# nikhilTkur/Multigrid_dolfinx

Measured on AMD Instinct MI355X. Metric: V-cycles/sec + achieved HBM GB/s, 3D Poisson P1 1024³ DoF, 1/2/4/8 MI355X, higher is better.
Workload: dtype f64; 1 GPU; 3D Poisson P1, 6-level 1024^3 fine grid, 1076890625 DoF, V(50,50) weighted Jacobi omega=0.6667, injection, Q1 prolongation, exact block-LU coarsest solve, explicit zeros pruned (7-point rows); levels=6, dim=3, elements_per_dim=1024, parallelism=single

## Files before the change

multigrid_dolfinx_amd/csrc/mg_capi.hip:

```cpp
#include "../../include/mg_hip.h"
#include "mg_csr_check.h"
#include "mg_kernels.hip.h"
#include "mg_direct.hip.h"
#include "mg_jacobi2.hip.h"
#include "mg_jacobik3d.hip.h"
#include "mg_jacobiblk.hip.h"
#include "mg_lattice.hip.h"
#include "mg_diffusion_mf.hip.h"
#include "mg_diffusion_mf_batch.hip.h"
#include "mg_diffusion_adj.hip.h"
#include "mg_diffusion_flux.hip.h"
#include "mg_diffusion_points.hip.h"
#include "mg_diffusion_kappa.hip.h"

#include <dlfcn.h>
#include <rccl/rccl.h>

#include <algorithm>
#include <array>
#include <cmath>
#include <cstdio>
#include <cstdlib>
#include <cstring>
#include <initializer_list>
// ... 121 lines not shown
    int64_t rep_escape = 0;
    int cls_halo = 0;
    bool flat = false;
    int W = 0, R = 1;
    int64_t nslices = 0;
    DevBuf<double> vals;
    DevBuf<int> cols;
    DevBuf<unsigned long long> codes;
    DevBuf<int> offsets;
    int ntable = 0, dcode = 0;
    bool coded = false;
    bool rb_ok = false;
    int mc_ok = -1;
    DevBuf<double> dvals;
    bool sdia = false;
    int wu = 0;
    int up[8] = {0, 0, 0, 0, 0, 0, 0, 0};
    int64_t mlead = 0, mslices = 0;
    DevBuf<unsigned char> cls;
    DevBuf<double> ctab;
    int ncls = 0;
    DevBuf<unsigned char> scls;
    DevBuf<int> s_off;
    DevBuf<double> s_val;
    DevBuf<int> s_cnt;
    int nscls = 0;
    DevBuf<int> s_pack;
    int lm_ntop = 0;
    int lm_top[LM_K] = {0, 0, 0, 0, 0, 0, 0, 0};
    struct MarchPlan {
        DevBuf<int> iv;
        int64_t waves[2] = {0, 0}, planes[2] = {0, 0};
    };
    MarchPlan plan[6];
    int cmain = 0;
    double cm[8] = {0, 0, 0, 0, 0, 0, 0, 0};
    int64_t cls_lead = 0;
    DevBuf<double> dinv;
    bool mf = false;
    DevBuf<double> kappa;
    int faces = MG_FACES_ALL;
    bool diffusion_hierarchy = false;
    bool react = false;
    DevBuf<double> rdiag;
    int robin = 0;
    DVector v, v2, f, err, ftrue;
    DVector sw;
    DVector fcg_x, fcg_p, fcg_q, fcg_b;
    bool cheb_est_ok = false;
    double cheb_lmax_est = 0.0, cheb_user_lmin = 0.0, cheb_user_lmax = 0.0;
    DevBuf<int> perm;
    int p1_ok = -1;
    std::vector<int> h_offsets;
    unsigned long long nnz_stored = 0, nnz_nonzero = 0;
    std::vector<int> splits;
};

}

struct DirectSolver {
    bool tried = false, ok = false;
    BtGeom g{};
    DevBuf<double> T;
    DevBuf<int> lcol, ucol;
    DevBuf<double> lval, uval;
    DevBuf<double> y, x, w;
};
// ... 76 lines not shown
    DevBuf<double> alpha[6];
    int alpha_N = 0;
    int dkappa_gather = 0;
    int lattice_tile = 0;
    int lattice_segments = 0;
    int slab_pair_form = 0;
    int graph_comm = 0;
    uint64_t epoch = 1;
    std::vector<CycleGraph> graphs;
    bool capturing = false;
    int use_direct = 1;
    int require_diagonal = 1;
    int fuse_restrict = 1;
    int fuse_block = 1;
    int64_t fuse_block_min_rows = (int64_t)1 << 15, fuse_block_max_rows = (int64_t)1 << 23;
    int fuse_block_k = 0, fuse_block_ez = 11;
    int direct_block_rows = 2048;
    int fuse_2d_lines = 0;
    int gen_odd_rows = 0;
    int cls_escape = 1;
    int storage_auto = 1;
    int storage_qbits = 0;
    int use_classes = 1;
    int fuse_sweeps = 1;
    int64_t fuse_min_rows = (int64_t)1 << 24;
    int fuse_segments = 0;
    int fuse_nontemporal = 0;
    int fuse_classes = 1;
    int fuse_plain_shape = 0;
    int fuse_plain = 2;
    int class_sweeps = 1;
    int fuse_k = 5;
    int fuse_k_shape = -1;
    int fuse_k_segments = 0;
    int timing_force_form = -1;
    int64_t fuse_k_slab_min_rows = (int64_t)1 << 20;
    int fuse_k_slab_min_sweeps = 4;
    int64_t fuse_k_min_rows = (int64_t)1 << 24;
    int64_t fuse_k_small_rows = (int64_t)1 << 22;
    int64_t fuse_k5_min_rows = (int64_t)1 << 26;
    int64_t fuse_k4_min_rows = 0;
    int fuse_k_nt_store = 0;
    int fuse_k_min_side = 32;
    int fuse_k_tail = 1;
    int fuse_k_small_tiles = 0;
    int fuse_k_pf = 1;
    int fuse_k_dpp = 1;
    int fuse_k_plan = 1;
    std::vector<const void*> large_lds_kernels;
    int fuse_shape = 1;
    int fuse_wi = 0;
    int fuse_even = 0;
    int march_sweeps = 1;
    int64_t march_min_rows = (int64_t)1 << 22;
    int march_shape = 0;
    int64_t fuse_small_2d_rows = 2048;
    int fuse_small = 1;
    int fuse_2d = 1;
    int fuse_2d_k = 5;
    int fuse_xcd_chunk = 32;
    int cls_blocks_per_cu = 4;
    DirectSolver direct;
    DevTemp ptab_count;
    int p1_prolong = 0;
    DevTemp rtab_count;
    DevTemp rtab_off;
// ... 1199 lines not shown
template <int K>
int escape_window_k(mg_context* c, const Level& L, const unsigned char* cls, int64_t clead, unsigned* most) {
    constexpr int WI = 64 - 2 * K, HY = 16 * 2 - 2 * K + 2;
    JK3WindowArgs a{};
    a.cls = cls; a.clead = clead; a.P = L.g.plane; a.nx = L.g.nx; a.ny = L.g.ny; a.nz = L.g.nk;
    a.ntx = (a.nx + WI - 1) / WI; a.nty = (a.ny + HY - 1) / HY;
    a.most = reinterpret_cast<unsigned*>(c->partials.get());
    HIP_TRY(hipMemsetAsync(a.most, 0, sizeof(unsigned), c->stream));
    hipLaunchKernelGGL((jk3_escape_window<K, 16, 2, 1>), dim3((unsigned)(a.ntx * a.nty)), dim3(256), 0, c->stream, a);
    HIP_TRY(hipGetLastError());
    HIP_TRY(hipMemcpyAsync(most, a.most, sizeof(unsigned), hipMemcpyDeviceToHost, c->stream));
    HIP_TRY(hipStreamSynchronize(c->stream));
    if (std::getenv("MG_DEBUG_STORAGE"))
        std::fprintf(stderr, "[mg] escape rows: at most %u in %d planes of a tile (%d sweeps per pass, pool of %d)\n", *most, K + 2, K, jk3_pool(K));
    return 0;
}

int escape_kmax(mg_context* c, const Level& L, const unsigned char* cls, int64_t clead, int* kmax) {
    *kmax = 0;
    if (L.wu != 4 || L.g.nk < 8 || L.g.nx < 32 || L.g.ny < 32) return 0;
    unsigned most = 0;
    MG_TRY(escape_window_k<5>(c, L, cls, clead, &most));
    if (most <= (unsigned)jk3_pool(5)) { *kmax = 5; return 0; }
    MG_TRY(escape_window_k<4>(c, L, cls, clead, &most));
    if (most <= (unsigned)jk3_pool(4)) { *kmax = 4; return 0; }
    MG_TRY(escape_window_k<3>(c, L, cls, clead, &most));
    if (most <= (unsigned)jk3_pool(3)) *kmax = 3;
    return 0;
}

struct JK3Range { int za0, za1, zb0, zb1; };

int jk3_shape(const mg_context* c, int K) {
    return c->fuse_k_shape >= 0 ? c->fuse_k_shape : (K >= 5 ? 8 : 7);
}

int jk3_shape_for(const mg_context* c, int K, int ncls) {
    return jk3_shape(c, K) >= 3 && ncls > 64 ? 1 : jk3_shape(c, K);
}

int march_plan_slot(const mg_context* c, const Level& L, int K) {
    if (!c->fuse_k_plan || !c->fuse_k_dpp || K < 3 || K > 5 || !L.cls || L.cls_escape || is_slab(c, L)) return -1;
    const int shape = jk3_shape_for(c, K, L.ncls);
    return shape == 7 || shape == 8 ? (K - 3) * 2 + (shape - 7) : -1;
}

int ensure_march_plan(mg_context* c, Level& L, int K, int slot) {
    Level::MarchPlan& mp = L.plan[slot];
    if (mp.iv) return 0;
    JK3PlanArgs a{};
    a.cls = L.cls; a.clead = L.cls_lead; a.P = L.g.plane; a.nx = L.g.nx; a.ny = L.g.ny; a.nz = L.g.nk; a.cmain = L.cmain;
    const int WI = 64 - 2 * K, HY = 32 - 2 * K + 2;
    a.ntx = (a.nx + WI - 1) / WI; a.nty = (a.ny + HY - 1) / HY;
    const size_t n = (size_t)a.ntx * a.nty * 16 * 4;
    DevBuf<int> iv;
    MG_TRY(iv.alloc(c, n));
    a.plan = iv;
    with_int<3, 4, 5>(K, [&](auto k) { hipLaunchKernelGGL((jk3_plan<decltype(k)::value, 16, 2, 1>), dim3((unsigned)(a.ntx * a.nty)), dim3(16 * WAVE), 0, c->stream, a); });
    HIP_TRY(hipGetLastError());
    std::vector<int> h(n);
    HIP_TRY(hipMemcpyAsync(h.data(), iv, n * sizeof(int), hipMemcpyDeviceToHost, c->stream));
    HIP_TRY(hipStreamSynchronize(c->stream));
    for (size_t i = 0; i < n; i += 4) {
        if (h[i + 1] > h[i]) { ++mp.waves[0]; mp.planes[0] += h[i + 1] - h[i]; }
        if (h[i + 3] > h[i + 2] && (h[i + 2] != h[i] || h[i + 3] != h[i + 1])) { ++mp.waves[1]; mp.planes[1] += h[i + 3] - h[i + 2]; }
    }
    mp.iv = std::move(iv);
    return 0;
}

template <int K, int NW, int LPW, int M, bool DPP, int PF = 1, int WPE = (NW == 12 ? 3 : 2), int TR = 256, bool ESC = false, bool B1 = false>
int launch_jacobikc_t(mg_context* c, JK3Args a, bool finest, const JK3Range& zr, int seglen) {
    constexpr int EX = 64 * M, EY = NW * LPW, WI = EX - 2 * K, HY = EY - 2 * K + 2;
    a.ntx = (a.nx + WI - 1) / WI;
    a.nty = (a.ny + HY - 1) / HY;
    const int64_t ntile = (int64_t)a.ntx * a.nty;
    constexpr size_t lds = B1 ? jk3b_lds_bytes<K, NW, LPW, M, TR>() : jk3_lds_bytes<K, NW, LPW, M, TR, ESC>();
    static_assert(lds <= 160 * 1024, "one CU's LDS");
    a.za0 = zr.za0; a.za1 = zr.za1; a.zb0 = zr.zb0; a.zb1 = zr.zb1;
    const int planes = std::max(0, zr.za1 - zr.za0) + std::max(0, zr.zb1 - zr.zb0);
    if (planes <= 0) return 0;
    a.ta = (int)ntile; a.seglen_b = 1;
    int64_t items = 0;
    if (seglen <= 0) {
        int64_t cus = std::max(1, c->prop.multiProcessorCount) * (int64_t)std::max<size_t>(1, std::min<size_t>(160 * 1024 / lds, (size_t)(4 * WPE / NW)));
        if (c->fuse_k_tail > 1) cus = c->fuse_k_tail;
        const double warm = 1.4 * K;
        int best = 1, best_ta = (int)ntile, best_m = 1;
        double best_cost = 1e300;
        const bool tail = c->fuse_k_tail && zr.zb1 <= zr.zb0;
        for (int n = 1; n <= std::max(1, planes / 8); ++n) {
            const int len = (planes + n - 1) / n;
            const int64_t full = ntile * n / cus;
            int64_t ta = tail ? std::min<int64_t>(ntile, full * cus / n) : ntile;
            if (ta <= 0 || (ntile - ta) * 2 > cus) ta = ntile;
            const int64_t tb = ntile - ta;
            const int m = tb > 0 ? (int)std::max<int64_t>(1, std::min<int64_t>(cus / tb, planes / 4)) : 1;
            const double cost = (double)((ta * n + cus - 1) / cus) * (len + warm) + (tb > 0 ? (planes + m - 1) / m + warm : 0.0);
            if (cost < best_cost) { best_cost = cost; best = n; best_ta = (int)ta; best_m = m; }
        }
        if (c->fuse_k_segments > 0) { best = std::min(c->fuse_k_segments, planes); best_ta = (int)ntile; }
        seglen = (planes + best - 1) / best;
        a.ta = best_ta;
        a.seglen_b = best_ta < ntile ? (planes + best_m - 1) / best_m : 1;
    }
    a.seglen = seglen;
    {
        const int nseg = (std::max(0, zr.za1 - zr.za0) + seglen - 1) / seglen + (std::max(0, zr.zb1 - zr.zb0) + seglen - 1) / seglen;
        items = (int64_t)a.ta * nseg;
        if (a.ta < ntile) items += (ntile - a.ta) * (int64_t)((planes + a.seglen_b - 1) / a.seglen_b);
    }
    a.xcd_chunk = (unsigned)c->fuse_xcd_chunk;
    unsigned grid = 0;
    MG_TRY(tile_grid(items, a.xcd_chunk, &grid));
    a.nitems = (unsigned)items;
    if (a.ncls > TR) return fail("more row classes than this tile shape keeps in LDS");
    void (*kern)(JK3Args) = nullptr;
    if constexpr (ESC) kern = sdia_jacobikc_escape<K, NW, LPW, M, DPP, PF, WPE, TR>;
    else if constexpr (B1) kern = finest ? sdia_jacobikc_finest_b1<K, NW, LPW, M, WPE, TR> : sdia_jacobikc_b1<K, NW, LPW, M, WPE, TR>;
    else kern = finest ? sdia_jacobikc_finest<K, NW, LPW, M, DPP, PF, WPE, TR> : sdia_jacobikc<K, NW, LPW, M, DPP, PF, WPE, TR>;
    MG_TRY(allow_large_lds(c, reinterpret_cast<const void*>(kern), lds));
    hipLaunchKernelGGL(kern, dim3(grid), dim3(NW * WAVE), lds, c->stream, a);
    HIP_TRY(hipGetLastError());
    c->jk3_tail = a.ta < ntile ? 1 : 0;
    return 0;
}

template <int K, int PF>
int launch_jacobikc_kp(mg_context* c, const JK3Args& a, bool finest, const JK3Range& zr, int seglen) {
    if (!c->fuse_k_dpp) return launch_jacobikc_t<K, 12, 2, 2, false, PF>(c, a, finest, zr, seglen);
    int shape = jk3_shape_for(c, K, a.ncls);
    if (shape == 1 && a.ncls <= 64 && K <= 4 && c->fuse_k_small_tiles) {
        constexpr int WI = 64 - 2 * K, HY = 48 - 2 * K + 2;
        if ((int64_t)((a.nx + WI - 1) / WI) * ((a.ny + HY - 1) / HY) < std::max(1, c->prop.multiProcessorCount)) shape = 4;
    }
    switch (shape) {
        case 1: return launch_jacobikc_t<K, 12, 4, 1, true, PF>(c, a, finest, zr, seglen);
        case 2: return launch_jacobikc_t<K, 8, 3, 2, true, PF>(c, a, finest, zr, seglen);
        case 3: return launch_jacobikc_t<K, 6, 4, 1, true, PF, 3, 64>(c, a, finest, zr, seglen);
        case 4: return launch_jacobikc_t<K, 8, 3, 1, true, PF, 4, 64>(c, a, finest, zr, seglen);
        case 5: if constexpr (K <= 4) return launch_jacobikc_t<K, 4, 6, 1, true, PF, 2, 64>(c, a, finest, zr, seglen);
        case 6: if constexpr (K <= 4 && PF == 1) return launch_jacobikc_t<K, 16, 3, 1, true, 1, 4>(c, a, finest, zr, seglen);
        case 7: return launch_jacobikc_t<K, 16, 2, 1, true, PF, 4>(c, a, finest, zr, seglen);
        case 8: if constexpr (PF == 1) return launch_jacobikc_t<K, 16, 2, 1, true, 1, 4, 256, false, true>(c, a, finest, zr, seglen);
                else return fail("tile shape 8 stages one plane of x (fuse_k_pf 1)");
        default: return launch_jacobikc_t<K, 12, 2, 2, true, PF>(c, a, finest, zr, seglen);
    }
}

template <int K>
int launch_jacobikc_k(mg_context* c, const JK3Args& a, bool finest, const JK3Range& zr, int seglen) {
    if (a.escape) {
        if constexpr (K >= 3) return launch_jacobikc_t<K, 16, 2, 1, true, 1, 4, 256, true>(c, a, finest, zr, seglen);
        else return fail("levels with escape rows take three to five sweeps per pass");
    }
    if constexpr (K == 3 || K == 4) {
        if (c->fuse_k_pf == 2 && (K == 3 || jk3_shape(c, K) == 7)) return launch_jacobikc_kp<K, 2>(c, a, finest, zr, seglen);
    }
    if constexpr (K == 2) return launch_jacobikc_t<K, 12, 4, 1, true, 1>(c, a, finest, zr, seglen);
    else return launch_jacobikc_kp<K, 1>(c, a, finest, zr, seglen);
}

int launch_jacobikc(mg_context* c, Level& L, int K, const double* x_rows, const double* f_rows, double* out_rows,
                    const JK3Range* zr = nullptr, int seglen = 0) {
    JK3Args a{};
    a.x = x_rows; a.f = f_rows; a.out = out_rows;
    fill_classes_lead(a, L);
    a.P = L.g.plane; a.nx = L.g.nx; a.ny = L.g.ny; a.nz = L.g.nk; a.omega = c->omega;
    const bool dist = is_slab(c, L);
    a.plo = dist && c->comm.rank > 0 ? K : 0;
    a.phi = dist && c->comm.rank + 1 < c->comm.world ? K : 0;
    if (dist && (L.hd < K || L.cls_halo != 1)) return fail("the level's halos are not prepared for that many sweeps per pass");
    if (L.cls_escape && K > L.esc_kmax) return fail("too many escape rows per tile for that many sweeps per pass");
    a.force_form = c->timing_force_form;
    a.nt_store = c->fuse_k_nt_store;
    if (const int slot = march_plan_slot(c, L, K); slot >= 0 && a.force_form < 0 && !zr) {
        if (!L.plan[slot].iv) {
            hipStreamCaptureStatus st = hipStreamCaptureStatusNone;
            HIP_TRY(hipStreamIsCapturing(c->stream, &st));
            if (st == hipStreamCaptureStatusNone) MG_TRY(ensure_march_plan(c, L, K, slot));
        }
        a.plan = L.plan[slot].iv;
    }
    a.escape = L.cls_escape ? 1 : 0; a.dvals = L.dvals; a.mlead = L.mlead; a.sshift = L.R == 1 ? 6 : (L.R == 2 ? 7 : 8);
    const JK3Range whole{0, L.g.nk, 0, 0};
    c->jk3_tail = 0;
    int rc = 0;
    if (!with_int<2, 3, 4, 5>(K, [&](auto k) { rc = launch_jacobikc_k<decltype(k)::value>(c, a, is_finest(c, L), zr ? *zr : whole, seglen); }))
        return fail("sweeps per pass must be in 2..5");
    return rc;
}

int check_coloring(mg_context* c, Level& L) {
    MG_TRY(need_stored_rows(c, L, "the colouring check of the Gauss-Seidel smoothers"));
    EllArgs a{};
    a.vals = L.vals; a.cols = L.cols; a.codes = L.codes; a.offsets = L.offsets; a.W = L.W;
    a.nloc = L.nloc; a.lead = L.g.lead; a.dinv = L.dinv; a.color_kind = COLOR_LATTICE9; a.grow0 = L.row0; a.gnx = L.g.nx; a.gny = L.g.ny;
    int* d_flag = reinterpret_cast<int*>(c->partials.get());
    HIP_TRY(hipMemsetAsync(d_flag, 0, sizeof(int), c->stream));
    const dim3 grid(blocks_for(L.nloc, 256)), blk(256);
    if (L.sdia) {
        a.vals = L.dvals; a.mlead = L.mlead;
        for (int t = 0; t < 8; ++t) a.up[t] = L.up[t];
        with_int_else<4, 1, 2>(L.R, [&](auto r) { hipLaunchKernelGGL(sdia_check_coloring<decltype(r)::value>, grid, blk, 0, c->stream, a, L.wu, d_flag); });
    } else {
        with_int_else<4, 1, 2>(L.R, [&](auto r) { hipLaunchKernelGGL(ell_check_coloring<decltype(r)::value>, grid, blk, 0, c->stream, a, L.nslices, d_flag); });
    }
    HIP_TRY(hipGetLastError());
    int flag = 1;
    HIP_TRY(hipMemcpyAsync(&flag, d_flag, sizeof(int), hipMemcpyDeviceToHost, c->stream));
    HIP_TRY(hipStreamSynchronize(c->stream));
    L.mc_ok = flag ? 0 : 1;
    return 0;
}

bool sweeps2d_ok(const mg_context* c, const Level& L) {
    if (!c->fuse_2d || !L.sdia || L.wu != 3 || !cls_full(L) || !c->fuse_classes || L.flat || !L.replicated) return false;
    return L.g.ny == 1 && L.up[1] == 1 && L.up[2] == L.g.nx && L.g.nx >= 8 && L.g.nz >= 8;
}

template <int K, int H>
// ... 2477 lines not shown
        c->lattice_march_min_rows = value;
    } else if (k == "dkappa_gather") {
        c->dkappa_gather = value != 0;
    } else if (k == "lattice_gs2") {
        c->lattice_gs2 = value != 0;
    } else if (k == "lattice_tile") {
        if (value < 0 || value > 2) return fail("lattice_tile must be 0, 1 or 2");
        c->lattice_tile = (int)value;
    } else if (k == "lattice_segments") {
        if (value < 0 || value > 4096) return fail("lattice_segments must be in 0..4096");
        c->lattice_segments = (int)value;
    } else if (k == "fuse_xcd_chunk") {
        if (value < 1 || value > 512) return fail("fuse_xcd_chunk must be in 1..512");
        c->fuse_xcd_chunk = (int)value;
    } else if (k == "cls_blocks_per_cu") {
        if (value < 1 || value > 64) return fail("cls_blocks_per_cu must be in 1..64");
        c->cls_blocks_per_cu = (int)value;
    } else if (k == "fuse_wi") {
        c->fuse_wi = (int)value;
    } else if (k == "fuse_even") {
        c->fuse_even = value != 0;
    } else if (k == "class_sweeps") {
        c->class_sweeps = value != 0;
    } else if (k == "fuse_plain_shape") {
        if (value < 0 || value > 2) return fail("fuse_plain_shape must be 0..2");
        c->fuse_plain_shape = (int)value;
    } else if (k == "fuse_plain") {
        if (value != 1 && value != 2) return fail("fuse_plain must be 1 or 2");
        c->fuse_plain = (int)value;
    } else if (k == "fuse_k") {
        if (value < 0 || value > 5) return fail("fuse_k must be in 0..5 (below 3: pairs of sweeps only)");
        c->fuse_k = (int)value;
    } else if (k == "fuse_k_shape") {
        if (value < -1 || value > 8) return fail("fuse_k_shape must be 0..8, or -1 (by sweeps per pass)");
        c->fuse_k_shape = (int)value;
    } else if (k == "fuse_k_slab_min_rows") {
        c->fuse_k_slab_min_rows = value;
    } else if (k == "fuse_k_slab_min_sweeps") {
        if (value < 2) return fail("fuse_k_slab_min_sweeps must be at least 2");
        c->fuse_k_slab_min_sweeps = (int)value;
    } else if (k == "fuse_k_min_rows") {
        c->fuse_k_min_rows = value;
    } else if (k == "fuse_k_small_rows") {
        c->fuse_k_small_rows = value;
    } else if (k == "fuse_k5_min_rows") {
        c->fuse_k5_min_rows = value;
    } else if (k == "fuse_k4_min_rows") {
        c->fuse_k4_min_rows = value;
    } else if (k == "fuse_k_nt_store") {
        c->fuse_k_nt_store = value != 0;
    } else if (k == "fuse_k_min_side") {
        if (value < 16 || value > 32) return fail("fuse_k_min_side must be in 16..32");
        c->fuse_k_min_side = (int)value;
    } else if (k == "fuse_k_tail") {
        if (value < 0) return fail("fuse_k_tail must be >= 0");
        c->fuse_k_tail = (int)value;
    } else if (k == "fuse_k_small_tiles") {
        c->fuse_k_small_tiles = value != 0;
    } else if (k == "fuse_k_pf") {
        if (value != 1 && value != 2) return fail("fuse_k_pf must be 1 or 2");
        c->fuse_k_pf = (int)value;
    } else if (k == "fuse_k_dpp") {
        c->fuse_k_dpp = value != 0;
    } else if (k == "fuse_k_plan") {
        c->fuse_k_plan = value != 0;
    } else if (k == "fuse_k_segments") {
        if (value < 0) return fail("fuse_k_segments must be >= 0");
        c->fuse_k_segments = (int)value;
    } else if (k == "fuse_classes") {
        c->fuse_classes = value != 0;
    } else if (k == "fuse_nontemporal") {
        c->fuse_nontemporal = value != 0;
    } else if (k == "fuse_segments") {
        if (value < 0) return fail("fuse_segments must be >= 0");
        c->fuse_segments = (int)value;
    } else if (k == "coarse_direct") {
        c->use_direct = value != 0;
        free_direct(c);
    } else if (k == "pcg_chunk") {
// ... 2102 lines not shown
```

multigrid_dolfinx_amd/csrc/mg_jacobik3d.hip.h:

```cpp
#pragma once
#include "mg_jacobi2.hip.h"
#include <type_traits>

namespace mgk {

struct JK3Args {
    const double* x;
    const double* f;
    double* out;
    const unsigned char* cls;
    const double* ctab;
    int64_t clead, P;
    int ncls, cmain;
    double cm[8];
    double omega;
    int nx, ny, nz;
    int plo, phi;
    int ntx, nty, seglen, za0, za1, zb0, zb1;
    int ta, seglen_b;
    unsigned nitems, xcd_chunk;
    int nt_store;
    int escape;
    const double* dvals;
    int64_t mlead;
// ... 652 lines not shown

    for (int k = z0 - 2 * K; k < z1; ++k) step(k, XA, CA, hyA, XB, CB, hyB);
}

template <int K, int NW, int LPW, int M, bool DPP, int PF, int WPE, int TR>
__global__ __attribute__((amdgpu_flat_work_group_size(NW * WAVE, NW * WAVE), amdgpu_waves_per_eu(WPE, WPE)))
void sdia_jacobikc(JK3Args a) {
    jk3_body<K, NW, LPW, M, DPP, PF, TR>(a);
}

template <int K, int NW, int LPW, int M, bool DPP, int PF, int WPE, int TR>
__global__ __attribute__((amdgpu_flat_work_group_size(NW * WAVE, NW * WAVE), amdgpu_waves_per_eu(WPE, WPE)))
void sdia_jacobikc_finest(JK3Args a) {
    jk3_body<K, NW, LPW, M, DPP, PF, TR>(a);
}

template <int K, int NW, int LPW, int M, int WPE, int TR>
__global__ __attribute__((amdgpu_flat_work_group_size(NW * WAVE, NW * WAVE), amdgpu_waves_per_eu(WPE, WPE)))
void sdia_jacobikc_b1(JK3Args a) {
    jk3_body<K, NW, LPW, M, true, 1, TR, false, true>(a);
}
template <int K, int NW, int LPW, int M, int WPE, int TR>
__global__ __attribute__((amdgpu_flat_work_group_size(NW * WAVE, NW * WAVE), amdgpu_waves_per_eu(WPE, WPE)))
void sdia_jacobikc_finest_b1(JK3Args a) {
    jk3_body<K, NW, LPW, M, true, 1, TR, false, true>(a);
}

template <int K, int NW, int LPW, int M, bool DPP, int PF, int WPE, int TR>
__global__ __attribute__((amdgpu_flat_work_group_size(NW * WAVE, NW * WAVE), amdgpu_waves_per_eu(WPE, WPE)))
void sdia_jacobikc_escape(JK3Args a) {
    jk3_body<K, NW, LPW, M, DPP, PF, TR, true>(a);
}

struct JK3WindowArgs {
    const unsigned char* cls;
    int64_t clead, P;
    int nx, ny, nz, ntx, nty;
    unsigned* most;
};

template <int K, int NW, int LPW, int M>
__global__ __launch_bounds__(256) void jk3_escape_window(JK3WindowArgs a) {
    constexpr int EX = 64 * M, EY = NW * LPW, WI = EX - 2 * K, HY = EY - 2 * K + 2, W = K + 2;
    __shared__ unsigned s_ring[W], s_plane;
    const int tiy = (int)(blockIdx.x / (unsigned)a.ntx), tix = (int)(blockIdx.x % (unsigned)a.ntx);
    const int tx0 = tix * WI - K, ty0 = tiy * HY - (K - 1), xcl = a.nx + 1 - tx0;
    unsigned win = 0u, best = 0u;
    for (int p = 0; p < a.nz; ++p) {
        if (threadIdx.x == 0) s_plane = 0u;
        __syncthreads();
        unsigned n = 0u;
        for (int i = threadIdx.x; i < EX * EY; i += 256) {
            const int ex = i % EX, line = ty0 + i / EX;
            if (ex > xcl || line < -2 || line > a.ny + 1) continue;
            const int64_t row = (int64_t)p * a.P + (int64_t)line * a.nx + tx0 + ex;
            n += a.cls[a.clead + row] == CLS_ESCAPE ? 1u : 0u;
        }
        if (n) atomicAdd(&s_plane, n);
        __syncthreads();
        if (threadIdx.x == 0) {
            win += s_plane - (p >= W ? s_ring[p % W] : 0u);
            s_ring[p % W] = s_plane;
            best = max(best, win);
        }
    }
    if (threadIdx.x == 0 && best) atomicMax(a.most, best);
}

struct JK3PlanArgs {
    const unsigned char* cls;
    int64_t clead, P;
    int nx, ny, nz, ntx, nty, cmain;
    int* plan;
};

template <int K, int NW, int LPW, int M>
__global__ __launch_bounds__(NW * WAVE) void jk3_plan(JK3PlanArgs a) {
    constexpr int EX = 64 * M, EY = NW * LPW, NC = M * LPW, WI = EX - 2 * K, HY = EY - 2 * K + 2;
    constexpr int U = 4;
    const int lane = threadIdx.x & 63;
    const int wave = __builtin_amdgcn_readfirstlane((int)(threadIdx.x >> 6));
    const unsigned tt = blockIdx.x;
    const int tiy = (int)(tt / (unsigned)a.ntx), tix = (int)(tt % (unsigned)a.ntx);
    const int tx0 = tix * WI - K, ty0 = tiy * HY - (K - 1);
    const int ey0 = wave * LPW, bias = 2 * a.nx + K + 2, xcl = a.nx + 1 - tx0;
    unsigned eo[NC];
#pragma unroll
    for (int c = 0; c < NC; ++c) eo[c] = jk3_cell_offset(ty0 + ey0 + c / M, lane + 64 * (c % M), a.nx, a.ny, tx0, xcl, bias);
    const unsigned char* const clsb = jk3_class_base(a.cls, a.clead, bias);
    int p0 = 0, p1 = 0, prun = 0;
    int q0 = 0, q1 = 0, qrun = 0;
    int prev[NC];
#pragma unroll
    for (int c = 0; c < NC; ++c) prev[c] = -1;
    for (int pb = 0; pb < a.nz; pb += U) {
        int cl[U][NC];
#pragma unroll
        for (int u = 0; u < U; ++u) {
            const unsigned char* const cb = clsb + (int64_t)min(pb + u, a.nz - 1) * a.P;
#pragma unroll
            for (int c = 0; c < NC; ++c) cl[u][c] = cb[eo[c] >> 3];
        }
#pragma unroll
        for (int u = 0; u < U; ++u) {
            const int p = pb + u;
            if (p >= a.nz) break;
            bool all = true, same = true;
#pragma unroll
            for (int c = 0; c < NC; ++c) {
                all = all && cl[u][c] == a.cmain;
                same = same && cl[u][c] == prev[c];
                prev[c] = cl[u][c];
            }
            if (__ballot(!all) != 0ull) {
                if (p - prun > p1 - p0) { p0 = prun; p1 = p; }
                prun = p + 1;
            }
            if (__ballot(!same) != 0ull) {
                if (p - qrun > q1 - q0) { q0 = qrun; q1 = p; }
                qrun = p;
            }
        }
    }
    if (a.nz - prun > p1 - p0) { p0 = prun; p1 = a.nz; }
    if (a.nz - qrun > q1 - q0) { q0 = qrun; q1 = a.nz; }
    if (lane == 0) {
        int* const pw = a.plan + 4 * ((int)tt * NW + wave);
        pw[0] = p0; pw[1] = p1; pw[2] = q0; pw[3] = q1;
    }
}

}
```

Baseline: 4.793 V-cycles/s.

## Add rim-line tile shape for five-sweep fused Jacobi on large levels

Adds tile shape 9 for the five-sweep temporally fused 3D Jacobi kernel. In this shape the first and last waves of a 16-wave block each own K-1 rim lines and the interior waves own two lines each, which makes the tile taller than the 32-line shape 8 while keeping one LDS x plane. It is selected by default for K=5 on levels with at least 2^26 rows, with its own march-plan slot and plan kernel, and the plan walk is factored into a shared helper. The intent is to cut halo recompute and redundant loads per output row. The cost is uneven work per wave, plus more LDS and register pressure from the per-wave line map.

```diff
diff --git a/multigrid_dolfinx_amd/csrc/mg_capi.hip b/multigrid_dolfinx_amd/csrc/mg_capi.hip
--- a/multigrid_dolfinx_amd/csrc/mg_capi.hip
+++ b/multigrid_dolfinx_amd/csrc/mg_capi.hip
@@ -177,7 +177,7 @@
         DevBuf<int> iv;
         int64_t waves[2] = {0, 0}, planes[2] = {0, 0};
     };
-    MarchPlan plan[6];
+    MarchPlan plan[7];
     int cmain = 0;
     double cm[8] = {0, 0, 0, 0, 0, 0, 0, 0};
     int64_t cls_lead = 0;
@@ -320,6 +320,7 @@
     int class_sweeps = 1;
     int fuse_k = 5;
     int fuse_k_shape = -1;
+    int64_t fuse_k_rim_min_rows = (int64_t)1 << 26;
     int fuse_k_segments = 0;
     int timing_force_form = -1;
     int64_t fuse_k_slab_min_rows = (int64_t)1 << 20;
@@ -1585,16 +1586,22 @@
 struct JK3Range { int za0, za1, zb0, zb1; };
 
 int jk3_shape(const mg_context* c, int K) {
-    return c->fuse_k_shape >= 0 ? c->fuse_k_shape : (K >= 5 ? 8 : 7);
-}
-
-int jk3_shape_for(const mg_context* c, int K, int ncls) {
-    return jk3_shape(c, K) >= 3 && ncls > 64 ? 1 : jk3_shape(c, K);
-}
-
+    const int shape = c->fuse_k_shape >= 0 ? c->fuse_k_shape : (K >= 5 ? 8 : 7);
+    return shape == 9 && K < 5 ? 7 : shape;
+}
+
+int jk3_shape_for(const mg_context* c, int K, int ncls, bool whole, int64_t rows) {
+    int shape = jk3_shape(c, K);
+    if (c->fuse_k_shape < 0 && K >= 5 && rows >= c->fuse_k_rim_min_rows) shape = 9;
+    if (shape >= 3 && ncls > 64) return 1;
+    return shape == 9 && !whole ? 8 : shape;
+}
+
+constexpr int MARCH_PLAN_SLOT_RIM = 6;
 int march_plan_slot(const mg_context* c, const Level& L, int K) {
     if (!c->fuse_k_plan || !c->fuse_k_dpp || K < 3 || K > 5 || !L.cls || L.cls_escape || is_slab(c, L)) return -1;
-    const int shape = jk3_shape_for(c, K, L.ncls);
+    const int shape = jk3_shape_for(c, K, L.ncls, true, L.nloc);
+    if (shape == 9) return MARCH_PLAN_SLOT_RIM;
     return shape == 7 || shape == 8 ? (K - 3) * 2 + (shape - 7) : -1;
 }
 
@@ -1603,13 +1610,15 @@
     if (mp.iv) return 0;
     JK3PlanArgs a{};
     a.cls = L.cls; a.clead = L.cls_lead; a.P = L.g.plane; a.nx = L.g.nx; a.ny = L.g.ny; a.nz = L.g.nk; a.cmain = L.cmain;
-    const int WI = 64 - 2 * K, HY = 32 - 2 * K + 2;
+    const bool rim = slot == MARCH_PLAN_SLOT_RIM;
+    const int WI = 64 - 2 * K, HY = rim ? jk3_rim_map<5>::HY : 32 - 2 * K + 2;
     a.ntx = (a.nx + WI - 1) / WI; a.nty = (a.ny + HY - 1) / HY;
     const size_t n = (size_t)a.ntx * a.nty * 16 * 4;
     DevBuf<int> iv;
     MG_TRY(iv.alloc(c, n));
     a.plan = iv;
-    with_int<3, 4, 5>(K, [&](auto k) { hipLaunchKernelGGL((jk3_plan<decltype(k)::value, 16, 2, 1>), dim3((unsigned)(a.ntx * a.nty)), dim3(16 * WAVE), 0, c->stream, a); });
+    if (rim) hipLaunchKernelGGL((jk3_plan_rim<5>), dim3((unsigned)(a.ntx * a.nty)), dim3(16 * WAVE), 0, c->stream, a);
+    else with_int<3, 4, 5>(K, [&](auto k) { hipLaunchKernelGGL((jk3_plan<decltype(k)::value, 16, 2, 1>), dim3((unsigned)(a.ntx * a.nty)), dim3(16 * WAVE), 0, c->stream, a); });
     HIP_TRY(hipGetLastError());
     std::vector<int> h(n);
     HIP_TRY(hipMemcpyAsync(h.data(), iv, n * sizeof(int), hipMemcpyDeviceToHost, c->stream));
@@ -1622,13 +1631,14 @@
     return 0;
 }
 
-template <int K, int NW, int LPW, int M, bool DPP, int PF = 1, int WPE = (NW == 12 ? 3 : 2), int TR = 256, bool ESC = false, bool B1 = false>
+template <int K, int NW, int LPW, int M, bool DPP, int PF = 1, int WPE = (NW == 12 ? 3 : 2), int TR = 256, bool ESC = false, bool B1 = false, bool RIM = false>
 int launch_jacobikc_t(mg_context* c, JK3Args a, bool finest, const JK3Range& zr, int seglen) {
-    constexpr int EX = 64 * M, EY = NW * LPW, WI = EX - 2 * K, HY = EY - 2 * K + 2;
+    static_assert(!RIM || (NW == jk3_rim_map<K>::NW && M == 1 && DPP && PF == 1 && WPE == 4 && !ESC && B1), "shape 9 is shape 8 with another line map");
+    constexpr int EX = 64 * M, EY = RIM ? jk3_rim_map<K>::EY : NW * LPW, WI = EX - 2 * K, HY = EY - 2 * K + 2;
     a.ntx = (a.nx + WI - 1) / WI;
     a.nty = (a.ny + HY - 1) / HY;
     const int64_t ntile = (int64_t)a.ntx * a.nty;
-    constexpr size_t lds = B1 ? jk3b_lds_bytes<K, NW, LPW, M, TR>() : jk3_lds_bytes<K, NW, LPW, M, TR, ESC>();
+    constexpr size_t lds = RIM ? jk3r_lds_bytes<K, TR>() : B1 ? jk3b_lds_bytes<K, NW, LPW, M, TR>() : jk3_lds_bytes<K, NW, LPW, M, TR, ESC>();
     static_assert(lds <= 160 * 1024, "one CU's LDS");
     a.za0 = zr.za0; a.za1 = zr.za1; a.zb0 = zr.zb0; a.zb1 = zr.zb1;
     const int planes = std::max(0, zr.za1 - zr.za0) + std::max(0, zr.zb1 - zr.zb0);
@@ -1670,6 +1680,7 @@
     if (a.ncls > TR) return fail("more row classes than this tile shape keeps in LDS");
     void (*kern)(JK3Args) = nullptr;
     if constexpr (ESC) kern = sdia_jacobikc_escape<K, NW, LPW, M, DPP, PF, WPE, TR>;
+    else if constexpr (RIM) kern = finest ? sdia_jacobikc_finest_rim<K, TR> : sdia_jacobikc_rim<K, TR>;
     else if constexpr (B1) kern = finest ? sdia_jacobikc_finest_b1<K, NW, LPW, M, WPE, TR> : sdia_jacobikc_b1<K, NW, LPW, M, WPE, TR>;
     else kern = finest ? sdia_jacobikc_finest<K, NW, LPW, M, DPP, PF, WPE, TR> : sdia_jacobikc<K, NW, LPW, M, DPP, PF, WPE, TR>;
     MG_TRY(allow_large_lds(c, reinterpret_cast<const void*>(kern), lds));
@@ -1680,9 +1691,9 @@
 }
 
 template <int K, int PF>
-int launch_jacobikc_kp(mg_context* c, const JK3Args& a, bool finest, const JK3Range& zr, int seglen) {
+int launch_jacobikc_kp(mg_context* c, const JK3Args& a, bool finest, const JK3Range& zr, int seglen, bool whole) {
     if (!c->fuse_k_dpp) return launch_jacobikc_t<K, 12, 2, 2, false, PF>(c, a, finest, zr, seglen);
-    int shape = jk3_shape_for(c, K, a.ncls);
+    int shape = jk3_shape_for(c, K, a.ncls, whole, a.P * a.nz);
     if (shape == 1 && a.ncls <= 64 && K <= 4 && c->fuse_k_small_tiles) {
         constexpr int WI = 64 - 2 * K, HY = 48 - 2 * K + 2;
         if ((int64_t)((a.nx + WI - 1) / WI) * ((a.ny + HY - 1) / HY) < std::max(1, c->prop.multiProcessorCount)) shape = 4;
@@ -1697,21 +1708,23 @@
         case 7: return launch_jacobikc_t<K, 16, 2, 1, true, PF, 4>(c, a, finest, zr, seglen);
         case 8: if constexpr (PF == 1) return launch_jacobikc_t<K, 16, 2, 1, true, 1, 4, 256, false, true>(c, a, finest, zr, seglen);
                 else return fail("tile shape 8 stages one plane of x (fuse_k_pf 1)");
+        case 9: if constexpr (K == 5 && PF == 1) return launch_jacobikc_t<K, 16, 2, 1, true, 1, 4, 64, false, true, true>(c, a, finest, zr, seglen);
+                else return fail("tile shape 9 takes five sweeps per pass and stages one plane of x");
         default: return launch_jacobikc_t<K, 12, 2, 2, true, PF>(c, a, finest, zr, seglen);
     }
 }
 
 template <int K>
-int launch_jacobikc_k(mg_context* c, const JK3Args& a, bool finest, const JK3Range& zr, int seglen) {
+int launch_jacobikc_k(mg_context* c, const JK3Args& a, bool finest, const JK3Range& zr, int seglen, bool whole) {
     if (a.escape) {
         if constexpr (K >= 3) return launch_jacobikc_t<K, 16, 2, 1, true, 1, 4, 256, true>(c, a, finest, zr, seglen);
         else return fail("levels with escape rows take three to five sweeps per pass");
     }
     if constexpr (K == 3 || K == 4) {
-        if (c->fuse_k_pf == 2 && (K == 3 || jk3_shape(c, K) == 7)) return launch_jacobikc_kp<K, 2>(c, a, finest, zr, seglen);
+        if (c->fuse_k_pf == 2 && (K == 3 || jk3_shape(c, K) == 7)) return launch_jacobikc_kp<K, 2>(c, a, finest, zr, seglen, whole);
     }
     if constexpr (K == 2) return launch_jacobikc_t<K, 12, 4, 1, true, 1>(c, a, finest, zr, seglen);
-    else return launch_jacobikc_kp<K, 1>(c, a, finest, zr, seglen);
+    else return launch_jacobikc_kp<K, 1>(c, a, finest, zr, seglen, whole);
 }
 
 int launch_jacobikc(mg_context* c, Level& L, int K, const double* x_rows, const double* f_rows, double* out_rows,
@@ -1739,7 +1752,7 @@
     const JK3Range whole{0, L.g.nk, 0, 0};
     c->jk3_tail = 0;
     int rc = 0;
-    if (!with_int<2, 3, 4, 5>(K, [&](auto k) { rc = launch_jacobikc_k<decltype(k)::value>(c, a, is_finest(c, L), zr ? *zr : whole, seglen); }))
+    if (!with_int<2, 3, 4, 5>(K, [&](auto k) { rc = launch_jacobikc_k<decltype(k)::value>(c, a, is_finest(c, L), zr ? *zr : whole, seglen, !dist); }))
         return fail("sweeps per pass must be in 2..5");
     return rc;
 }
@@ -4283,7 +4296,7 @@
         if (value < 0 || value > 5) return fail("fuse_k must be in 0..5 (below 3: pairs of sweeps only)");
         c->fuse_k = (int)value;
     } else if (k == "fuse_k_shape") {
-        if (value < -1 || value > 8) return fail("fuse_k_shape must be 0..8, or -1 (by sweeps per pass)");
+        if (value < -1 || value > 9) return fail("fuse_k_shape must be 0..9, or -1 (by sweeps per pass)");
         c->fuse_k_shape = (int)value;
     } else if (k == "fuse_k_slab_min_rows") {
         c->fuse_k_slab_min_rows = value;
@@ -4296,6 +4309,8 @@
         c->fuse_k_small_rows = value;
     } else if (k == "fuse_k5_min_rows") {
         c->fuse_k5_min_rows = value;
+    } else if (k == "fuse_k_rim_min_rows") {
+        c->fuse_k_rim_min_rows = value;
     } else if (k == "fuse_k4_min_rows") {
         c->fuse_k4_min_rows = value;
     } else if (k == "fuse_k_nt_store") {
diff --git a/multigrid_dolfinx_amd/csrc/mg_jacobik3d.hip.h b/multigrid_dolfinx_amd/csrc/mg_jacobik3d.hip.h
--- a/multigrid_dolfinx_amd/csrc/mg_jacobik3d.hip.h
+++ b/multigrid_dolfinx_amd/csrc/mg_jacobik3d.hip.h
@@ -708,6 +708,430 @@
     jk3_body<K, NW, LPW, M, DPP, PF, TR, true>(a);
 }
 
+template <int K> struct jk3_rim_map {
+    static constexpr int NW = 16, RL = K - 1;
+    static constexpr int NLM = RL > 2 ? RL : 2;
+    static constexpr int EY = 2 * RL + 2 * (NW - 2), HY = EY - 2 * K + 2, WI = 64 - 2 * K;
+    static constexpr int first(int wave) { return wave == 0 ? 0 : wave == NW - 1 ? EY - RL : RL + 2 * (wave - 1); }
+    static constexpr int lines(int wave) { return wave == 0 || wave == NW - 1 ? RL : 2; }
+};
+template <int K, int KIND> struct jk3_rim_kind {
+    static constexpr int NL = KIND == 0 ? 2 : K - 1;
+    static constexpr int cap(int l) { return KIND == 0 ? K : KIND == 1 ? l + 1 : K - 1 - l; }
+};
+
+template <int K, int TR> constexpr size_t jk3r_lds_bytes() {
+    return sizeof(double) * (TR * CLS_W + (size_t)(2 * (K - 1) * (jk3_rim_map<K>::EY + 1) + 1) * 64);
+}
+
+template <int K, int TR>
+__device__ __forceinline__ void jk3_rim_body(const JK3Args& a) {
+    using MAP = jk3_rim_map<K>;
+    constexpr int EX = 64, NW = MAP::NW, EY = MAP::EY, NCM = MAP::NLM, WI = MAP::WI, HY = MAP::HY;
+    constexpr int IS = (EY + 1) * EX, PS = (K - 1) * IS;
+    static_assert(CLS_W == 8, "table rows of eight doubles");
+    static_assert(K >= 3 && NCM <= 4, "a wave's class bytes of a plane live in one register");
+    static_assert(NCM * (K + 1) <= 64, "the fast-path flags live in one scalar register pair");
+    static_assert(8 * ((K - 2) * IS + (NCM + 1) * EX) < 65536, "every LDS access of a step is `register + 16-bit immediate`");
+    extern __shared__ double j2_smem[];
+    double* const sT = j2_smem;
+    const int lane = threadIdx.x & 63;
+    const int wave = __builtin_amdgcn_readfirstlane((int)(threadIdx.x >> 6));
+
+    unsigned id;
+    {
+        const unsigned b = blockIdx.x, xcd = b & 7u, j = b >> 3, ch = a.xcd_chunk;
+        id = ((j / ch) * 8u + xcd) * ch + (j % ch);
+    }
+    if (id >= a.nitems) return;
+    const unsigned ntile = (unsigned)(a.ntx * a.nty);
+    const int nsa = (a.za1 - a.za0 + a.seglen - 1) / a.seglen;
+    const int nsb = (a.zb1 - a.zb0 + a.seglen - 1) / a.seglen;
+    const unsigned items_a = (unsigned)a.ta * (unsigned)(nsa + max(nsb, 0));
+    unsigned tt;
+    int z0, z1;
+    if (id < items_a) {
+        const int seg = (int)(id / (unsigned)a.ta);
+        tt = id % (unsigned)a.ta;
+        z0 = seg < nsa ? a.za0 + seg * a.seglen : a.zb0 + (seg - nsa) * a.seglen;
+        z1 = min(seg < nsa ? a.za1 : a.zb1, z0 + a.seglen);
+    } else {
+        const unsigned j = id - items_a, tb = ntile - (unsigned)a.ta;
+        tt = (unsigned)a.ta + j % tb;
+        z0 = a.za0 + (int)(j / tb) * a.seglen_b;
+        z1 = min(a.za1, z0 + a.seglen_b);
+    }
+    const int tiy = (int)(tt / (unsigned)a.ntx), tix = (int)(tt % (unsigned)a.ntx);
+    if (z1 <= z0) return;
+    const int tx0 = tix * WI - K, ty0 = tiy * HY - (K - 1);
+
+    {
+        const int nt = a.ncls * CLS_W;
+        for (int i = threadIdx.x; i < nt; i += NW * WAVE) {
+            double v = a.ctab[i];
+            if ((i & (CLS_W - 1)) == CLS_W - 1) {
+                const double d = a.ctab[i - 4];
+                v = a.omega * (1.0 / (d != 0.0 ? d : 1.0));
+            }
+            sT[i] = v;
+        }
+        constexpr int NZ = (2 * (K - 1) * (EY + 1) + 1) * EX;
+        for (int i = threadIdx.x; i < NZ; i += NW * WAVE) sT[TR * CLS_W + i] = 0.0;
+    }
+    const double m0 = a.cm[0], m1 = a.cm[1], m2 = a.cm[2], m3 = a.cm[3], m4 = a.cm[4], m5 = a.cm[5], m6 = a.cm[6];
+    const double mcf = a.omega * (1.0 / (m3 != 0.0 ? m3 : 1.0));
+    const int cmain = a.cmain;
+
+    const int ey0 = MAP::first(wave);
+    const int wkind = wave == 0 ? 1 : wave == NW - 1 ? 2 : 0;
+    int bcur = 0, bprev = 0;
+    int lbase = TR * CLS_W + ey0 * EX + lane;
+    asm volatile("" : "+v"(lbase));
+    auto limg = [&](int base, int t) -> double* { return j2_smem + base + (t - 1) * IS + EX; };
+    unsigned inT = 0;
+#pragma unroll
+    for (int l = 0; l < NCM; ++l) {
+        const int ey = ey0 + l;
+        if (lane >= K && lane < EX - K && ey >= K - 1 && ey <= EY - K && tx0 + lane < a.nx && ty0 + ey < a.ny) inT |= 1u << l;
+    }
+    auto shof = [&](int l) -> int {
+        const int64_t r = (int64_t)(ty0 + ey0 + l) * a.nx + (tx0 + (lbase & 63));
+        return r < 0 ? -1 : (r >= a.P ? 1 : 0);
+    };
+
+    const int bias = 2 * a.nx + K + 2;
+    const int xcl = a.nx + 1 - tx0;
+    unsigned eo[NCM];
+#pragma unroll
+    for (int l = 0; l < NCM; ++l) {
+        eo[l] = jk3_cell_offset(ty0 + ey0 + l, lane, a.nx, a.ny, tx0, xcl, bias);
+        asm volatile("" : "+v"(eo[l]));
+    }
+    const unsigned eos = jk3_cell_offset(ty0 + ey0 - 1, lane, a.nx, a.ny, tx0, xcl, bias);
+    const unsigned eon = jk3_cell_offset(ty0 + ey0 + MAP::lines(wave), lane, a.nx, a.ny, tx0, xcl, bias);
+    const unsigned char* const clsb = jk3_class_base(a.cls, a.clead, bias);
+    const double* const xb0 = a.x - bias;
+    const double* const fb0 = a.f - bias;
+    auto sbase = [](const void* p) -> gcptr_t {
+        const unsigned long long u = (unsigned long long)p;
+        const unsigned lo = (unsigned)__builtin_amdgcn_readfirstlane((int)(unsigned)u);
+        const unsigned hi = (unsigned)__builtin_amdgcn_readfirstlane((int)(unsigned)(u >> 32));
+        return (gcptr_t)(((unsigned long long)hi << 32) | lo);
+    };
+    auto ldd = [](gcptr_t b, unsigned e8) -> double {
+        asm volatile("" : "+v"(e8));
+        return *(const __attribute__((address_space(1))) double*)(b + e8);
+    };
+    typedef unsigned int __attribute__((aligned(1))) u32_unaligned_t;
+    auto ldc = [](gcptr_t b, unsigned e8) -> int {
+        unsigned e = e8 >> 3;
+        asm volatile("" : "+v"(e));
+        return (int)*(const __attribute__((address_space(1))) u32_unaligned_t*)(b + e);
+    };
+    const int pmin = -a.plo - 1, pmax = a.nz + a.phi;
+
+    int klo = 0x7fffffff, khi = 0x7fffffff, kform = 0;
+    if (a.plan) {
+        const int* const pw = a.plan + 4 * ((int)tt * NW + wave);
+        const int top = a.nz - K - 1;
+        const int lo0 = max(max(pw[0], 1), z0 - K), hi0 = min(pw[1] - K, top);
+        const int lo1 = max(max(pw[2], 1), z0 - K), hi1 = min(pw[3] - K, top);
+        const int n0 = min(hi0, z1) - lo0, n1 = min(hi1, z1) - lo1;
+        if (n0 > 0 && n0 >= n1) {
+            klo = __builtin_amdgcn_readfirstlane(lo0);
+            khi = __builtin_amdgcn_readfirstlane(hi0);
+        } else if (n1 > 0) {
+            klo = __builtin_amdgcn_readfirstlane(lo1);
+            khi = __builtin_amdgcn_readfirstlane(hi1);
+            kform = 1;
+        }
+    }
+    auto interior_step = [&](int k) -> bool { return k >= klo && k < khi; };
+
+    double acc[K][NCM], fr[K][NCM], X[NCM], XP[NCM], hS = 0.0, hN = 0.0;
+    int C[NCM];
+    unsigned cw[K + 1];
+    unsigned long long fast = 0;
+#pragma unroll
+    for (int l = 0; l < NCM; ++l) {
+#pragma unroll
+        for (int t = 0; t < K; ++t) acc[t][l] = fr[t][l] = 0.0;
+        X[l] = XP[l] = 0.0;
+        C[l] = 0;
+    }
+#pragma unroll
+    for (int j = 0; j <= K; ++j) cw[j] = 0u;
+
+    auto load_slice = [&](auto kind, const int i, const int n, const int plane, const int fplane, const bool noc) __attribute__((always_inline)) {
+        constexpr int NL = decltype(kind)::NL;
+        const int64_t o = (int64_t)min(max(plane, pmin), pmax) * a.P;
+        const gcptr_t cb = sbase(clsb + o);
+        const gcptr_t xb = sbase(xb0 + o);
+        const gcptr_t fb = sbase(fb0 + (int64_t)min(max(fplane, pmin), pmax) * a.P);
+#pragma unroll
+        for (int l = 0; l < NL; ++l) {
+            if ((l * n) / NL != i) continue;
+            X[l] = ldd(xb, eo[l]);
+            if (!noc) C[l] = ldc(cb, eo[l]);
+            fr[K - 1][l] = ldd(fb, eo[l]);
+        }
+        if (i == n - 1) { hS = ldd(xb, eos); hN = ldd(xb, eon); }
+    };
+    auto cls_of = [&](int j, int l) -> int { return (int)((cw[j] >> (8 * l)) & 255u); };
+    auto cls_now = [&](int j, int l) -> int {
+        unsigned w = cw[j];
+        asm volatile("" : "+v"(w));
+        return (int)((w >> (8 * l)) & 255u);
+    };
+    int k_plane = 0;
+    bool k_store = false;
+    __attribute__((address_space(1))) char* k_out = nullptr;
+    auto store = [&](int l, double v) {
+        unsigned e8 = eo[l];
+        asm volatile("" : "+v"(e8));
+        if (a.nt_store) __builtin_nontemporal_store(v, (__attribute__((address_space(1))) double*)(k_out + e8));
+        else *(__attribute__((address_space(1))) double*)(k_out + e8) = v;
+    };
+    int lo_t[K + 1], n_t[K + 1];
+#pragma unroll
+    for (int t = 1; t <= K; ++t) {
+        lo_t[t] = -min(a.plo, K - t);
+        n_t[t] = a.nz + min(a.phi, K - t) - lo_t[t];
+    }
+
+    auto phase_a_fast = [&](auto col_tag, auto kind) __attribute__((always_inline)) {
+        constexpr bool COL = decltype(col_tag)::value;
+        using KD = decltype(kind);
+#pragma unroll
+        for (int l = 0; l < KD::NL; ++l) {
+            const int iw = l * EX;
+            double k0 = m0, k6 = m6, kcf = mcf;
+            if constexpr (COL) {
+                const dvec2_t* const tr = reinterpret_cast<const dvec2_t*>(sT + CLS_W * cls_of(0, l));
+                const dvec2_t t01 = tr[0], t67 = tr[3];
+                k0 = t01.x; k6 = t67.x; kcf = t67.y;
+            }
+            double nw = X[l];
+#pragma unroll
+            for (int t = 1; t <= K; ++t) {
+                if (t > KD::cap(l)) {
+                    if (t == KD::cap(l) + 1) limg(bcur, t - 1)[iw] = nw;
+                    continue;
+                }
+                const double wd = t == 1 ? XP[l] : limg(bprev, t - 1)[iw];
+                const double s = fma(k6, nw, acc[t - 1][l]);
+                const double o = wd + kcf * (fr[K - t][l] - s);
+                acc[t - 1][l] = fma(k0, wd, 0.0);
+                if (t > 1) limg(bcur, t - 1)[iw] = nw;
+                nw = o;
+            }
+            if (KD::cap(l) == K && k_store && (inT >> l & 1u)) store(l, nw);
+        }
+    };
+    auto phase_b_fast = [&](auto col_tag, auto kind, const int t) __attribute__((always_inline)) {
+        constexpr bool COL = decltype(col_tag)::value;
+        using KD = decltype(kind);
+        constexpr int NL = KD::NL;
+        const double* const img = limg(bcur, t > 1 ? t - 1 : 1);
+        double v[NL], ys, yn;
+        if (t == 1) {
+            ys = hS;
+#pragma unroll
+            for (int l = 0; l < NL; ++l) v[l] = X[l];
+            yn = hN;
+        } else {
+            ys = img[-EX];
+#pragma unroll
+            for (int l = 0; l < NL; ++l) v[l] = img[l * EX];
+            yn = img[NL * EX];
+        }
+#pragma unroll
+        for (int l = 0; l < NL; ++l) {
+            if (t > KD::cap(l)) continue;
+            const double yw = jk3_from_west(v[l]), ye = jk3_from_east(v[l]);
+            double k1 = m1, k2 = m2, k3 = m3, k4 = m4, k5 = m5;
+            if constexpr (COL) {
+                const dvec2_t* const tr = reinterpret_cast<const dvec2_t*>(sT + CLS_W * cls_of(0, l));
+                const dvec2_t t01 = tr[0], t23 = tr[1], t45 = tr[2];
+                k1 = t01.y; k2 = t23.x; k3 = t23.y; k4 = t45.x; k5 = t45.y;
+            }
+            double s = acc[t - 1][l];
+            s = fma(k1, l > 0 ? v[l > 0 ? l - 1 : 0] : ys, s);
+            s = fma(k2, yw, s);
+            s = fma(k3, v[l], s);
+            s = fma(k4, ye, s);
+            s = fma(k5, l + 1 < NL ? v[l + 1 < NL ? l + 1 : l] : yn, s);
+            acc[t - 1][l] = s;
+        }
+    };
+    auto phase_a_general = [&](auto kind) __attribute__((always_inline)) {
+        using KD = decltype(kind);
+#pragma unroll
+        for (int l = 0; l < KD::NL; ++l) {
+            const int iw = l * EX;
+            double nw = X[l];
+            int pc = k_plane + shof(l);
+            asm volatile("" : "+v"(pc));
+#pragma unroll
+            for (int t = 1; t <= K; ++t) {
+                const int j = K - t;
+                double* const img = limg(bcur, t > 1 ? t - 1 : 1);
+                if (t > KD::cap(l)) {
+                    if (t == KD::cap(l) + 1) img[iw] = nw;
+                    continue;
+                }
+                const double wd = t == 1 ? XP[l] : limg(bprev, t - 1)[iw];
+                const dvec2_t t67 = reinterpret_cast<const dvec2_t*>(sT + CLS_W * cls_now(j, l))[3];
+                const dvec2_t t01 = reinterpret_cast<const dvec2_t*>(sT + CLS_W * cls_now(j + 1, l))[0];
+                const double s = fma(t67.x, nw, acc[t - 1][l]);
+                double o = wd + t67.y * (fr[j][l] - s);
+                o = (unsigned)(pc + j - lo_t[t]) < (unsigned)n_t[t] ? o : 0.0;
+                acc[t - 1][l] = fma(t01.x, wd, 0.0);
+                if (t > 1) img[iw] = nw;
+                nw = o;
+                __builtin_amdgcn_sched_barrier(0);
+            }
+            if (KD::cap(l) == K && k_store && (inT >> l & 1u)) store(l, nw);
+        }
+    };
+    auto phase_b_general = [&](auto kind, const int t) __attribute__((always_inline)) {
+        using KD = decltype(kind);
+        constexpr int NL = KD::NL;
+        double x0w[NL], x0e[NL];
+        if (t == 1) {
+#pragma unroll
+            for (int l = 0; l < NL; ++l) { x0w[l] = jk3_from_west(X[l]); x0e[l] = jk3_from_east(X[l]); }
+        }
+#pragma unroll
+        for (int l = 0; l < NL; ++l) {
+            if (t > KD::cap(l)) continue;
+            const int iw = l * EX;
+            double ys, yw, yd, ye, yn;
+            if (t == 1) {
+                ys = l > 0 ? X[l > 0 ? l - 1 : l] : hS;
+                yw = x0w[l]; yd = X[l]; ye = x0e[l];
+                yn = l + 1 < NL ? X[l + 1 < NL ? l + 1 : l] : hN;
+            } else {
+                const double* const img = limg(bcur, t - 1);
+                ys = img[iw - EX]; yw = img[iw - 1]; yd = img[iw]; ye = img[iw + 1]; yn = img[iw + EX];
+            }
+            const dvec2_t* const tr = reinterpret_cast<const dvec2_t*>(sT + CLS_W * cls_now(K - t, l));
+            const dvec2_t t01 = tr[0], t23 = tr[1], t45 = tr[2];
+            double s = acc[t - 1][l];
+            s = fma(t01.y, ys, s);
+            s = fma(t23.x, yw, s);
+            s = fma(t23.y, yd, s);
+            s = fma(t45.x, ye, s);
+            s = fma(t45.y, yn, s);
+            acc[t - 1][l] = s;
+            __builtin_amdgcn_sched_barrier(0);
+        }
+    };
+
+    auto step = [&](auto kind, const int k) __attribute__((always_inline)) {
+        using KD = decltype(kind);
+        constexpr int NL = KD::NL;
+        constexpr unsigned long long ALLFAST = (1ull << (NL * (K + 1))) - 1ull;
+        k_plane = k; k_store = k >= z0;
+        bcur = lbase + (k & 1) * PS;
+        bprev = lbase + ((k + 1) & 1) * PS;
+        asm volatile("" : "+v"(bcur));
+        asm volatile("" : "+v"(bprev));
+        {
+            const unsigned long long u = (unsigned long long)(a.out - bias + (int64_t)k * a.P);
+            const unsigned lo = (unsigned)__builtin_amdgcn_readfirstlane((int)(unsigned)u);
+            const unsigned hi = (unsigned)__builtin_amdgcn_readfirstlane((int)(unsigned)(u >> 32));
+            k_out = (__attribute__((address_space(1))) char*)(((unsigned long long)hi << 32) | lo);
+        }
+#pragma unroll
+        for (int l = 0; l < NL; ++l) asm volatile("" : "+v"(X[l]));
+        const bool interior = interior_step(k);
+        if (k == khi) {
+            unsigned m = 0;
+#pragma unroll
+            for (int l = 0; l < NL; ++l)
+                if (__builtin_amdgcn_readfirstlane((int)(__ballot(cls_of(0, l) != cmain) == 0ull))) m |= 1u << l;
+            fast = 0;
+#pragma unroll
+            for (int j = 0; j < K; ++j) {
+                fast |= (unsigned long long)m << (j * NL);
+                cw[j] = cw[0];
+            }
+        }
+        int form = kform;
+        if (!interior) {
+            unsigned m = 0;
+            cw[K] = 0u;
+#pragma unroll
+            for (int l = 0; l < NL; ++l) {
+                asm volatile("" : "+v"(C[l]));
+                C[l] &= 255;
+                cw[K] |= (unsigned)C[l] << (8 * l);
+                if (__builtin_amdgcn_readfirstlane((int)(__ballot(C[l] != cmain) == 0ull))) m |= 1u << l;
+            }
+            fast |= (unsigned long long)m << (K * NL);
+            form = 2;
+            if ((a.plo > 0 || k >= 1) && (a.phi > 0 || k + K + 1 < a.nz)) {
+                if (fast == ALLFAST) {
+                    form = 0;
+                } else {
+                    bool same = true;
+#pragma unroll
+                    for (int j = 1; j <= K; ++j) same = same && cw[j] == cw[0];
+                    if (__builtin_amdgcn_readfirstlane((int)(__ballot(!same) == 0ull))) form = 1;
+                }
+            }
+        }
+        if (a.force_form >= 0) form = a.force_form;
+        if (form == 0) phase_a_fast(std::false_type{}, kind);
+        else if (form == 1) phase_a_fast(std::true_type{}, kind);
+        else phase_a_general(kind);
+#pragma unroll
+        for (int l = 0; l < NL; ++l) XP[l] = X[l];
+#pragma unroll
+        for (int l = 0; l < NL; ++l) {
+#pragma unroll
+            for (int j = 0; j + 1 < K; ++j) fr[j][l] = fr[j + 1][l];
+            if (KD::cap(l) >= 2) asm volatile("" : "+v"(fr[K - 2][l]));
+        }
+        if (!interior) {
+#pragma unroll
+            for (int j = 0; j < K; ++j) cw[j] = cw[j + 1];
+            fast >>= NL;
+        }
+        __syncthreads();
+#pragma unroll
+        for (int t = 1; t <= K; ++t) {
+            if (form == 0) phase_b_fast(std::false_type{}, kind, t);
+            else if (form == 1) phase_b_fast(std::true_type{}, kind, t);
+            else phase_b_general(kind, t);
+            __builtin_amdgcn_sched_barrier(0);
+            load_slice(kind, t - 1, K, k + K + 1, k + K, interior_step(k + 1));
+            __builtin_amdgcn_sched_barrier(0);
+        }
+    };
+
+    auto march = [&](auto kind) __attribute__((always_inline)) {
+        load_slice(kind, 0, 1, z0 - K, z0 - K - 1, false);
+        __syncthreads();
+        for (int k = z0 - 2 * K; k < z1; ++k) step(kind, k);
+    };
+    if (wkind == 0) march(jk3_rim_kind<K, 0>{});
+    else if (wkind == 1) march(jk3_rim_kind<K, 1>{});
+    else march(jk3_rim_kind<K, 2>{});
+}
+
+template <int K, int TR>
+__global__ __attribute__((amdgpu_flat_work_group_size(16 * WAVE, 16 * WAVE), amdgpu_waves_per_eu(4, 4)))
+void sdia_jacobikc_rim(JK3Args a) {
+    jk3_rim_body<K, TR>(a);
+}
+template <int K, int TR>
+__global__ __attribute__((amdgpu_flat_work_group_size(16 * WAVE, 16 * WAVE), amdgpu_waves_per_eu(4, 4)))
+void sdia_jacobikc_finest_rim(JK3Args a) {
+    jk3_rim_body<K, TR>(a);
+}
+
 struct JK3WindowArgs {
     const unsigned char* cls;
     int64_t clead, P;
@@ -750,10 +1174,52 @@
     int* plan;
 };
 
+template <int NC>
+__device__ __forceinline__ void jk3_plan_walk(const JK3PlanArgs& a, const unsigned char* const clsb, const unsigned (&eo)[NC], int* const pw) {
+    constexpr int U = 4;
+    const int lane = threadIdx.x & 63;
+    int p0 = 0, p1 = 0, prun = 0;
+    int q0 = 0, q1 = 0, qrun = 0;
+    int prev[NC];
+#pragma unroll
+    for (int c = 0; c < NC; ++c) prev[c] = -1;
+    for (int pb = 0; pb < a.nz; pb += U) {
+        int cl[U][NC];
+#pragma unroll
+        for (int u = 0; u < U; ++u) {
+            const unsigned char* const cb = clsb + (int64_t)min(pb + u, a.nz - 1) * a.P;
+#pragma unroll
+            for (int c = 0; c < NC; ++c) cl[u][c] = cb[eo[c] >> 3];
+        }
+#pragma unroll
+        for (int u = 0; u < U; ++u) {
+            const int p = pb + u;
+            if (p >= a.nz) break;
+            bool all = true, same = true;
+#pragma unroll
+            for (int c = 0; c < NC; ++c) {
+                all = all && cl[u][c] == a.cmain;
+                same = same && cl[u][c] == prev[c];
+                prev[c] = cl[u][c];
+            }
+            if (__ballot(!all) != 0ull) {
+                if (p - prun > p1 - p0) { p0 = prun; p1 = p; }
+                prun = p + 1;
+            }
+            if (__ballot(!same) != 0ull) {
+                if (p - qrun > q1 - q0) { q0 = qrun; q1 = p; }
+                qrun = p;
+            }
+        }
+    }
+    if (a.nz - prun > p1 - p0) { p0 = prun; p1 = a.nz; }
+    if (a.nz - qrun > q1 - q0) { q0 = qrun; q1 = a.nz; }
+    if (lane == 0) { pw[0] = p0; pw[1] = p1; pw[2] = q0; pw[3] = q1; }
+}
+
 template <int K, int NW, int LPW, int M>
 __global__ __launch_bounds__(NW * WAVE) void jk3_plan(JK3PlanArgs a) {
     constexpr int EX = 64 * M, EY = NW * LPW, NC = M * LPW, WI = EX - 2 * K, HY = EY - 2 * K + 2;
-    constexpr int U = 4;
     const int lane = threadIdx.x & 63;
     const int wave = __builtin_amdgcn_readfirstlane((int)(threadIdx.x >> 6));
     const unsigned tt = blockIdx.x;
@@ -763,47 +1229,22 @@
     unsigned eo[NC];
 #pragma unroll
     for (int c = 0; c < NC; ++c) eo[c] = jk3_cell_offset(ty0 + ey0 + c / M, lane + 64 * (c % M), a.nx, a.ny, tx0, xcl, bias);
-    const unsigned char* const clsb = jk3_class_base(a.cls, a.clead, bias);
-    int p0 = 0, p1 = 0, prun = 0;
-    int q0 = 0, q1 = 0, qrun = 0;
-    int prev[NC];
-#pragma unroll
-    for (int c = 0; c < NC; ++c) prev[c] = -1;
-    for (int pb = 0; pb < a.nz; pb += U) {
-        int cl[U][NC];
-#pragma unroll
-        for (int u = 0; u < U; ++u) {
-            const unsigned char* const cb = clsb + (int64_t)min(pb + u, a.nz - 1) * a.P;
-#pragma unroll
-            for (int c = 0; c < NC; ++c) cl[u][c] = cb[eo[c] >> 3];
-        }
-#pragma unroll
-        for (int u = 0; u < U; ++u) {
-            const int p = pb + u;
-            if (p >= a.nz) break;
-            bool all = true, same = true;
-#pragma unroll
-            for (int c = 0; c < NC; ++c) {
-                all = all && cl[u][c] == a.cmain;
-                same = same && cl[u][c] == prev[c];
-                prev[c] = cl[u][c];
-            }
-            if (__ballot(!all) != 0ull) {
-                if (p - prun > p1 - p0) { p0 = prun; p1 = p; }
-                prun = p + 1;
-            }
-            if (__ballot(!same) != 0ull) {
-                if (p - qrun > q1 - q0) { q0 = qrun; q1 = p; }
-                qrun = p;
-            }
-        }
-    }
-    if (a.nz - prun > p1 - p0) { p0 = prun; p1 = a.nz; }
-    if (a.nz - qrun > q1 - q0) { q0 = qrun; q1 = a.nz; }
-    if (lane == 0) {
-        int* const pw = a.plan + 4 * ((int)tt * NW + wave);
-        pw[0] = p0; pw[1] = p1; pw[2] = q0; pw[3] = q1;
-    }
-}
-
-}
+    jk3_plan_walk<NC>(a, jk3_class_base(a.cls, a.clead, bias), eo, a.plan + 4 * ((int)tt * NW + wave));
+}
+
+template <int K>
+__global__ __launch_bounds__(16 * WAVE) void jk3_plan_rim(JK3PlanArgs a) {
+    using MAP = jk3_rim_map<K>;
+    const int lane = threadIdx.x & 63;
+    const int wave = __builtin_amdgcn_readfirstlane((int)(threadIdx.x >> 6));
+    const unsigned tt = blockIdx.x;
+    const int tiy = (int)(tt / (unsigned)a.ntx), tix = (int)(tt % (unsigned)a.ntx);
+    const int tx0 = tix * MAP::WI - K, ty0 = tiy * MAP::HY - (K - 1);
+    const int ey0 = MAP::first(wave), nl = MAP::lines(wave), bias = 2 * a.nx + K + 2, xcl = a.nx + 1 - tx0;
+    unsigned eo[MAP::NLM];
+#pragma unroll
+    for (int l = 0; l < MAP::NLM; ++l) eo[l] = jk3_cell_offset(ty0 + ey0 + min(l, nl - 1), lane, a.nx, a.ny, tx0, xcl, bias);
+    jk3_plan_walk<MAP::NLM>(a, jk3_class_base(a.cls, a.clead, bias), eo, a.plan + 4 * ((int)tt * MAP::NW + wave));
+}
+
+}
```

Result: faster. 4.988 V-cycles/s (median of 6 runs) (+4.1%).
